# openfheorg/openfhe-development

Measured on AMD Instinct MI355X. Metric: NTT GB/s vs HBM roofline + CKKS EvalMultKeySwitch/sec, N=2^16 L=30, 1/2/4/8 GPU, higher is better.
Workload: dtype u64; 1 GPU; batched fwd+inv negacyclic NTT, N=2^16, L=30 x 60-bit limbs, 1024 polynomials per GPU (BASELINE configs[1]); global_batch=1024, parallelism=batch-sharded x1, no data-path collective

## Files before the change

### openfhe-development_amd/csrc/fhe_hip.cpp

```cpp
#include "../../include/fhe_hip.h"

#include <algorithm>
#include <cmath>
#include <cstdio>
#include <cstdlib>
#include <map>
#include <mutex>
#include <shared_mutex>
#include <string>
#include <vector>

#include "basis_kernels.h"
#include "bfv_kernels.h"
#include "elemwise_kernels.h"
#include "host_math.h"
#include "ntt_kernels.h"
#include "ntt_static.h"
#include "ntt_row8.h"
#include "rt.h"
#include "sampler_kernels.h"
#include "blake2_kernels.h"

using namespace fhe;

static thread_local std::string g_lastError;
static fhe_status fail(fhe_status code, const std::string& msg) {
    g_lastError = msg;
    return code;
}
#define RT_CHECK(expr)                                                                  \
    do {                                                                                \
        const char* _e = (expr);                                                        \
        if (_e)                                                                         \
            return fail(FHE_ERR_DEVICE, std::string(#expr) + ": " + _e);                \
    } while (0)
#define ARG_CHECK(cond, msg)                  \
    do {                                      \
        if (!(cond))                          \
            return fail(FHE_ERR_ARG, msg);    \
    } while (0)

extern "C" const char* fhe_last_error(void) { return g_lastError.c_str(); }
extern "C" const char* fhe_version(void) {
#ifdef FHE_EMU
    return "fhe_hip 0.1 (TEST lane emulator build — not a product build)";
#else
    return "fhe_hip 0.1 (gfx950)";
#endif
}
extern "C" int fhe_device_count(void) { return rt::device_count(); }

namespace fhe {
namespace host {
bool is_prime(uint64_t n) {
    static const uint64_t w[] = {2, 3, 5, 7, 11, 13, 17, 19, 23, 29, 31, 37};
    if (n < 2)
        return false;
    for (uint64_t p : w) {
        if (n == p)
            return true;
        if (n % p == 0)
            return false;
    }
    uint64_t d = n - 1;
    int s      = 0;
    while (!(d & 1)) {
        d >>= 1;
        ++s;
    }
    for (uint64_t a : w) {
        uint64_t x = powmod(a, d, n);
// ... 559 lines not shown
}
static fhe_status launch_pass(const fhe_ctx* c, const PassPlan& pp, bool inverse, const uint64_t* xin, uint64_t* xout,
                              const LimbSel& sel, uint32_t nLimbs, uint32_t batch, bool canonOut, void* stream,
                              uint32_t inStride = 0, uint32_t inFirst = 0, uint32_t outStride = 0, uint32_t outFirst = 0,
                              const NttEpilogue* epi = nullptr, const uint32_t* proSrcLimb = nullptr, int64_t inDelta = 0) {
    NttPassArgs a;
    const uint32_t grid = fill_pass_args(c, pp, inverse, xin, xout, sel, nLimbs, batch, canonOut, inStride, inFirst, outStride,
                                         outFirst, a);
    if (inDelta) {
        if (c->logN < (uint32_t)kTileLog)
            return fail(FHE_ERR_UNSUPPORTED, "ntt: separately allocated towers need a ring of at least 4096");
        a.inDelta = inDelta;
    }
    if (proSrcLimb) {
        a.proMode = 1, a.proSrcLimb = *proSrcLimb;
        const int mode = static_mode(c, pp, inverse);
        if (pp.layoutA && !inverse && mode == 1 && pp.T == 4)
            FHE_LAUNCH_BARRIER((ntt_static_kernel<true, false, 4, 1, false, true>), grid, stream, a);
        else if (pp.layoutA && !inverse && mode == 1 && pp.T == 5)
            FHE_LAUNCH_BARRIER((ntt_static_kernel<true, false, 5, 1, false, true>), grid, stream, a);
        else
            return fail(FHE_ERR_UNSUPPORTED, "ntt: no prologue kernel for this pass shape");
        LAUNCH_CHECK();
        return FHE_OK;
    }
    if (epi && epi->mode) {
        a.epiMode = epi->mode, a.epiSplit = epi->split, a.epiAStride = epi->aStride, a.epiAFirst = epi->aFirst;
        a.epiA = epi->A, a.epiC = epi->C, a.epiOut0 = epi->out0, a.epiOut1 = epi->out1;
        a.epiADelta = epi->aDelta;
        const int mode = static_mode(c, pp, inverse);
        bool launched  = false;
#define FHE_EPI_CASE(TT, MODE) \
    if (!launched && !pp.layoutA && !inverse && pp.T == TT && mode == MODE) { \
        FHE_LAUNCH_BARRIER((ntt_static_kernel<false, false, TT, MODE, true>), grid, stream, a); \
        launched = true; \
    }
        FHE_EPI_CASE(12, 9) FHE_EPI_CASE(11, 9) FHE_EPI_CASE(10, 9) FHE_EPI_CASE(9, 9) FHE_EPI_CASE(12, 1)
#undef FHE_EPI_CASE
        if (!launched)
            return fail(FHE_ERR_UNSUPPORTED, "ntt: no epilogue kernel for this pass shape");
        LAUNCH_CHECK();
        return FHE_OK;
    }
    if (c->logN >= (uint32_t)kTileLog) {
        const int mode = static_mode(c, pp, inverse);
        bool launched  = false;
#define FHE_STATIC_CASE(LA, INV, TT, MODE) \
    if (!launched && pp.layoutA == LA && inverse == INV && pp.T == TT && mode == MODE) { \
        FHE_LAUNCH_BARRIER((ntt_static_kernel<LA, INV, TT, MODE>), grid, stream, a); \
        launched = true; \
    }
        if (!pp.layoutA && c->logN > (uint32_t)kTileLog && row8_for(pp.T)) {
            const uint32_t rgrid = a.rows << (c->logN - pp.T);
            a.xcdSwizzle         = ((nLimbs << (c->logN - pp.T)) % 8u == 0) ? 1u : 0u;
#define FHE_ROW8_CASE(INV, TT, MODE) \
    if (!launched && inverse == INV && pp.T == TT && mode == MODE) { \
        FHE_LAUNCH_BARRIER_N((r8::ntt_row8_kernel<INV, TT - 9, MODE>), rgrid, 64u << (TT - 9), stream, a); \
        launched = true; \
    }
            FHE_ROW8_CASE(false, 12, 9) FHE_ROW8_CASE(true, 12, 0) FHE_ROW8_CASE(false, 11, 9) FHE_ROW8_CASE(true, 11, 0)
            FHE_ROW8_CASE(false, 10, 9) FHE_ROW8_CASE(true, 10, 0) FHE_ROW8_CASE(false, 9, 9) FHE_ROW8_CASE(true, 9, 0)
#undef FHE_ROW8_CASE
        }
        FHE_STATIC_CASE(true, false, 4, 1) FHE_STATIC_CASE(true, true, 4, 1)
        FHE_STATIC_CASE(true, false, 5, 1) FHE_STATIC_CASE(true, true, 5, 1)
        FHE_STATIC_CASE(false, false, 12, 9) FHE_STATIC_CASE(false, true, 12, 0)
        FHE_STATIC_CASE(false, false, 11, 9) FHE_STATIC_CASE(false, true, 11, 0)
        FHE_STATIC_CASE(false, false, 10, 9) FHE_STATIC_CASE(false, true, 10, 0)
        FHE_STATIC_CASE(false, false, 9, 9) FHE_STATIC_CASE(false, true, 9, 0)
        FHE_STATIC_CASE(false, false, 12, 1) FHE_STATIC_CASE(false, true, 12, 1)
#undef FHE_STATIC_CASE
        if (!launched)
            return fail(FHE_ERR_UNSUPPORTED, "ntt: no kernel instance for this pass shape");
        LAUNCH_CHECK();
        return FHE_OK;
    }
    if (pp.layoutA) {
        if (inverse)
            FHE_LAUNCH_BARRIER((ntt_pass_kernel<true, true>), grid, stream, a);
        else
            FHE_LAUNCH_BARRIER((ntt_pass_kernel<true, false>), grid, stream, a);
    }
    else {
        if (inverse)
            FHE_LAUNCH_BARRIER((ntt_pass_kernel<false, true>), grid, stream, a);
        else
            FHE_LAUNCH_BARRIER((ntt_pass_kernel<false, false>), grid, stream, a);
    }
    LAUNCH_CHECK();
    return FHE_OK;
}

static uint32_t env_u32(const char* name, uint32_t dflt) {
    const char* v = std::getenv(name);
    return v ? (uint32_t)std::strtoul(v, nullptr, 10) : dflt;
}
static uint32_t ntt_t1(uint32_t logN) {
    const uint32_t dflt = std::max(4u, logN - (uint32_t)kTileLog);
    static const uint32_t forced = env_u32("FHE_NTT_T1", 0);
    if (forced >= 4 && forced <= 5 && logN > (uint32_t)kTileLog && logN - forced >= 9 && logN - forced <= 12)
        return forced;
    return dflt;
}

static bool ntt_epilogue_supported(const fhe_ctx* c) {
    if (c->logN < (uint32_t)kTileLog)
        return false;
    if (c->logN == (uint32_t)kTileLog)
        return true;
    const uint32_t t1 = ntt_t1(c->logN), t2 = c->logN - t1;
    return t2 == 12u || (t1 == 4u && t2 >= 9u && t2 <= 12u);
}
static bool ntt_prologue_supported(const fhe_ctx* c) {
    return c->logN > (uint32_t)kTileLog && ntt_t1(c->logN) <= 5u;
}
static fhe_status ntt_run(fhe_ctx* c, bool inverse, const uint64_t* xin, uint64_t* xout, const uint32_t* limbIdx,
                          uint32_t nLimbs, uint32_t batch, void* stream, uint32_t inStride = 0, uint32_t inFirst = 0,
                          uint32_t outStride = 0, uint32_t outFirst = 0, const NttEpilogue* epi = nullptr,
                          bool canonOut = true, const uint32_t* proSrcLimb = nullptr, int64_t inDelta = 0) {
    ARG_CHECK(c && xin && xout, "fhe_ntt: null argument");
    ARG_CHECK(batch >= 1, "fhe_ntt: batch must be >= 1");
    LimbSel sel;
    if (fhe_status s = make_sel(c, limbIdx, nLimbs, &sel, "fhe_ntt"))
        return s;
    RT_CHECK(rt::set_device(c->device));
    const uint32_t logN = c->logN;
    if (logN <= (uint32_t)kTileLog) {
        PassPlan p;
        plan_pass(inverse, false, logN, logN, &p);
        uint32_t bound = 1;
        mark_uniform(p, logN);
        if (!inverse)
            schedule_fwd(p, logN, &bound);
        p.outBound = bound;
        return launch_pass(c, p, inverse, xin, xout, sel, nLimbs, batch, canonOut, stream, inStride, inFirst, outStride, outFirst, epi,
                           nullptr, inDelta);
    }
    const uint32_t T1 = ntt_t1(logN), T2 = logN - T1;
    PassPlan pa, pb;
    plan_pass(inverse, true, logN, T1, &pa);
    plan_pass(inverse, false, logN, T2, &pb);
    mark_uniform(pa, logN);
    mark_uniform(pb, logN);
    if (!inverse) {
        uint32_t bound = 1;
        schedule_fwd(pa, logN, &bound);
        schedule_fwd(pb, logN, &bound);
        pb.outBound = bound;
    }
    const PassPlan& p1 = inverse ? pb : pa;
    const PassPlan& p2 = inverse ? pa : pb;
    if (fhe_status s = launch_pass(c, p1, inverse, xin, xout, sel, nLimbs, batch, false, stream, inStride, inFirst, outStride, outFirst,
                                   nullptr, proSrcLimb, inDelta))
        return s;
    return launch_pass(c, p2, inverse, xout, xout, sel, nLimbs, batch, canonOut, stream, outStride, outFirst, outStride, outFirst, epi);
}

extern "C" fhe_status fhe_ntt_fwd(fhe_ctx* c, uint64_t* x, const uint32_t* li, uint32_t nl, uint32_t b, void* st) {
    return ntt_run(c, false, x, x, li, nl, b, st);
}
extern "C" fhe_status fhe_ntt_inv(fhe_ctx* c, uint64_t* x, const uint32_t* li, uint32_t nl, uint32_t b, void* st) {
    return ntt_run(c, true, x, x, li, nl, b, st);
}
extern "C" fhe_status fhe_ntt_fwd_oop(fhe_ctx* c, const uint64_t* xi, uint64_t* xo, const uint32_t* li, uint32_t nl,
                                      uint32_t b, void* st) {
    return ntt_run(c, false, xi, xo, li, nl, b, st);
}
extern "C" fhe_status fhe_ntt_inv_oop(fhe_ctx* c, const uint64_t* xi, uint64_t* xo, const uint32_t* li, uint32_t nl,
                                      uint32_t b, void* st) {
    return ntt_run(c, true, xi, xo, li, nl, b, st);
}

extern "C" size_t fhe_poly_mul_workspace_bytes(const fhe_ctx* c, uint32_t nLimbs, uint32_t batch) {
    return c ? (((size_t)2 * batch * nLimbs) << c->logN) * 8 : 0;
}
static bool poly_mul_fused_supported(const fhe_ctx* c) {
    if (c->logN <= (uint32_t)kTileLog)
        return false;
    const uint32_t t1 = ntt_t1(c->logN), t2 = c->logN - t1;
    return (t1 == 4u && t2 >= 9u && t2 <= 12u) || (t1 == 5u && t2 == 12u);
}
extern "C" fhe_status fhe_poly_mul(fhe_ctx* c, const uint64_t* a, const uint64_t* b, uint64_t* out, const uint32_t* limbIdx,
                                   uint32_t nLimbs, uint32_t batch, void* wsv, size_t wsBytes, void* stream) {
    ARG_CHECK(c && a && b && out && wsv, "fhe_poly_mul: null argument");
    ARG_CHECK(batch >= 1, "fhe_poly_mul: batch must be >= 1");
    ARG_CHECK(wsBytes >= fhe_poly_mul_workspace_bytes(c, nLimbs, batch), "fhe_poly_mul: workspace too small");
    LimbSel sel;
    if (fhe_status s = make_sel(c, limbIdx, nLimbs, &sel, "fhe_poly_mul"))
        return s;
    RT_CHECK(rt::set_device(c->device));
    uint64_t* wa = (uint64_t*)wsv;
    uint64_t* wb = wa + (((size_t)batch * nLimbs) << c->logN);
    if (!poly_mul_fused_supported(c)) {
        if (fhe_status s = ntt_run(c, false, a, wa, limbIdx, nLimbs, batch, stream))
            return s;
        if (fhe_status s = ntt_run(c, false, b, wb, limbIdx, nLimbs, batch, stream))
            return s;
        if (fhe_status s = fhe_mul(c, out, wa, wb, limbIdx, nLimbs, batch, stream))
            return s;
        return ntt_run(c, true, out, out, limbIdx, nLimbs, batch, stream);
    }
    const uint32_t logN = c->logN, T1 = ntt_t1(logN), T2 = logN - T1;
    PassPlan fa, fb, ib, ia;
    plan_pass(false, true, logN, T1, &fa);
    plan_pass(false, false, logN, T2, &fb);
    plan_pass(true, false, logN, T2, &ib);
    plan_pass(true, true, logN, T1, &ia);
// ... 1028 lines not shown
    w.dig.assign(numParts, 0);
    size_t off = 0;
    w.coef = off, off += (size_t)batch * sizeQl * N;
    for (uint32_t j = 0; j < numParts; ++j) {
        const uint32_t start = p->alpha * j;
        const uint32_t sz    = (j == numParts - 1) ? sizeQl - start : p->alpha;
        w.dig[j] = off, off += (size_t)batch * (sizeQl - sz + p->sizeP) * N;
    }
    w.e0 = off, off += (size_t)batch * (sizeQl + p->sizeP) * N;
    w.e1 = off, off += (size_t)batch * (sizeQl + p->sizeP) * N;
    w.md = off, off += (size_t)2 * batch * sizeQl * N;
    w.pcoef = off, off += (size_t)2 * batch * p->sizeP * N;
    w.d2 = off, off += (size_t)batch * sizeQl * N;
    w.k0 = off, off += (size_t)batch * sizeQl * N;
    w.k1 = off, off += (size_t)batch * sizeQl * N;
    w.total = off;
    return w;
}
extern "C" size_t fhe_ks_workspace_bytes(const fhe_ks_plan* p, uint32_t sizeQl, uint32_t batch) {
    if (!p || sizeQl < 1 || sizeQl > p->sizeQ || batch < 1)
        return 0;
    return ks_layout(p, sizeQl, batch).total * 8;
}

static fhe_status mod_down_core(fhe_ks_plan* p, fhe_ks_plan::Level* lv, const uint64_t* x, uint32_t nTow, uint64_t* pcoef,
                                uint64_t* md, void* st, fhe_conv* down = nullptr, const NttEpilogue* epi = nullptr) {
    fhe_ctx* c            = p->ctx;
    const uint32_t sizeQl = lv->sizeQl, sizeP = p->sizeP, sizeQlP = sizeQl + sizeP;
    std::vector<uint32_t> pIdx(sizeP);
    for (uint32_t j = 0; j < sizeP; ++j)
        pIdx[j] = p->sizeQ + j;
    if (fhe_status s = ntt_run(c, true, x, pcoef, pIdx.data(), sizeP, nTow, st, sizeQlP, sizeQl))
        return s;
    if (fhe_status s = fhe_approx_switch_basis(down ? down : lv->down, pcoef, sizeP, 0, md, sizeQl, 0, nTow, st))
        return s;
    return ntt_run(c, false, md, md, nullptr, sizeQl, nTow, st, 0, 0, 0, 0, epi);
}
static fhe_status mod_down_tail(fhe_ks_plan* p, fhe_ks_plan::Level* lv, const uint64_t* x, const uint64_t* md, uint32_t nTow,
                                uint64_t* out, bool accumulate, void* st) {
    const uint32_t sizeQl = lv->sizeQl, sizeQlP = sizeQl + p->sizeP;
    if (accumulate)
        return elem_run<OP_SUB_MUL_CONST_ACC>(p->ctx, out, x, md, lv->d_PInv, nullptr, sizeQl, nTow, st, "fhe_approx_mod_down",
                                              sizeQlP, 0);
    return elem_run<OP_SUB_MUL_CONST>(p->ctx, out, x, md, lv->d_PInv, nullptr, sizeQl, nTow, st, "fhe_approx_mod_down", sizeQlP, 0);
}
static fhe_status mod_down_run(fhe_ks_plan* p, fhe_ks_plan::Level* lv, const uint64_t* x, uint32_t nTow, uint64_t* out,
                               uint64_t* pcoef, uint64_t* md, void* st) {
    if (fhe_status s = mod_down_core(p, lv, x, nTow, pcoef, md, st))
        return s;
    return mod_down_tail(p, lv, x, md, nTow, out, false, st);
}

static fhe_status ks_precompute_run(fhe_ks_plan* p, fhe_ks_plan::Level* lv, const uint64_t* cin, uint32_t batch,
                                    uint64_t* ws, const KsLayout& w, void* st) {
    fhe_ctx* c            = p->ctx;
    const uint32_t sizeQl = lv->sizeQl;
    if (fhe_status s = fhe_ntt_inv_oop(c, cin, ws + w.coef, nullptr, sizeQl, batch, st))
        return s;
    for (uint32_t j = 0; j < lv->numParts; ++j) {
        const uint32_t nc = (uint32_t)lv->cidx[j].size();
        uint64_t* dj      = ws + w.dig[j];
        if (fhe_status s = fhe_approx_switch_basis(lv->up[j], ws + w.coef, sizeQl, p->alpha * j, dj, nc, 0, batch, st))
            return s;
        if (fhe_status s = ntt_run(c, false, dj, dj, lv->cidx[j].data(), nc, batch, st, 0, 0, 0, 0, nullptr, false))
            return s;
    }
    return FHE_OK;
}
static fhe_status ks_inner_multi_launch(fhe_ks_plan* p, fhe_ks_plan::Level* lv, const fhe_ks_key* const* keys, uint32_t nKeys,
                                        const uint64_t* cin, uint32_t batch, uint64_t* const* e0, uint64_t* const* e1,
                                        const uint64_t* first, const TwPair* dP, uint64_t* ws, const KsLayout& w, void* st,
                                        uint32_t towOff = 0) {
    fhe_ctx* c            = p->ctx;
    const uint32_t sizeQl = lv->sizeQl, sizeP = p->sizeP, sizeQlP = sizeQl + sizeP;
    const uint32_t tilesPerRow = c->N >= (uint32_t)kTile ? (c->N >> kTileLog) : 1u;
    for (uint32_t t0 = 0; t0 < nKeys; t0 += (uint32_t)kMaxMultiKeys) {
        KsInnerMultiArgs g;
        const uint32_t nt = std::min<uint32_t>(kMaxMultiKeys, nKeys - t0);
        for (uint32_t j = 0; j < (uint32_t)kMaxDigits; ++j) {
            g.nc[j]     = j < lv->numParts ? (uint32_t)lv->cidx[j].size() : 0u;
            g.digits[j] = j < lv->numParts ? ws + w.dig[j] + (((size_t)towOff * g.nc[j]) << c->logN) : nullptr;
        }
        for (uint32_t t = 0; t < (uint32_t)kMaxMultiKeys; ++t) {
            const uint32_t tt = t < nt ? t0 + t : t0;
            g.keyB[t] = keys[tt]->d_b, g.keyA[t] = keys[tt]->d_a, g.out0[t] = e0[tt], g.out1[t] = e1[tt];
        }
        g.c = cin + (((size_t)towOff * sizeQl) << c->logN), g.first = first, g.firstC = dP;
        g.lc = c->d_lc, g.mu128 = c->d_mu128, g.red = c->d_red;
        g.logN = c->logN, g.batch = batch, g.sizeQl = sizeQl, g.sizeQ = p->sizeQ, g.sizeP = sizeP;
        g.numDigits = lv->numParts, g.alpha = p->alpha, g.nKeys = nt;
        const uint64_t grid = (((uint64_t)tilesPerRow * sizeQlP + 7) / 8) * 8 * batch;
        static const uint32_t ksm = env_u32("FHE_KSM", 1);
        uintptr_t bits = (uintptr_t)g.c | (uintptr_t)g.first;
        for (uint32_t j = 0; j < lv->numParts && j < (uint32_t)kMaxDigits; ++j)
            bits |= (uintptr_t)g.digits[j];
        for (uint32_t t = 0; t < nt; ++t)
            bits |= (uintptr_t)g.keyB[t] | (uintptr_t)g.keyA[t] | (uintptr_t)g.out0[t] | (uintptr_t)g.out1[t];
        const bool wide = (bits & 15u) == 0 && c->N >= 2;
        if (lv->numParts <= 3 && ksm == 1 && wide)
            FHE_LAUNCH((ks_inner_multi_kernel<3, 2, true>), grid, st, g);
        else if (lv->numParts <= 3 && ksm == 2 && wide)
            FHE_LAUNCH((ks_inner_multi_kernel<3, 2, false>), grid, st, g);
        else if (lv->numParts <= 3 && ksm == 3)
            FHE_LAUNCH((ks_inner_multi_kernel<3, 1, false>), grid, st, g);
        else if (lv->numParts <= 3)
            FHE_LAUNCH((ks_inner_multi_kernel<3>), grid, st, g);
        else if (lv->numParts <= 4)
            FHE_LAUNCH((ks_inner_multi_kernel<4>), grid, st, g);
        else
            FHE_LAUNCH((ks_inner_multi_kernel<8>), grid, st, g);
        LAUNCH_CHECK();
    }
    return FHE_OK;
}
static fhe_status ks_inner_run(fhe_ks_plan* p, fhe_ks_plan::Level* lv, const fhe_ks_key* key, const uint64_t* cin,
                               uint32_t batch, uint64_t* e0, uint64_t* e1, uint64_t* ws, const KsLayout& w, void* st,
                               uint32_t towOff = 0) {
// ... 19 lines not shown
    }
    return FHE_OK;
}
static fhe_status ks_inner_multi_run(fhe_ks_plan* p, fhe_ks_plan::Level* lv, const fhe_ks_key* const* keys, uint32_t nKeys,
                                     const uint64_t* cin, uint32_t batch, uint64_t* const* e0, uint64_t* const* e1,
                                     const uint64_t* first, const TwPair* dP, uint64_t* ws, const KsLayout& w, void* st) {
    if (lv->numParts <= (uint32_t)kMaxDigits)
        return ks_inner_multi_launch(p, lv, keys, nKeys, cin, batch, e0, e1, first, dP, ws, w, st);
    const uint32_t sizeQl = lv->sizeQl, sizeQlP = sizeQl + p->sizeP;
    for (uint32_t t = 0; t < nKeys; ++t) {
        if (fhe_status s = ks_inner_run(p, lv, keys[t], cin, batch, e0[t], e1[t], ws, w, st))
            return s;
        if (first)
            if (fhe_status s = elem_run<OP_MUL_CONST_ADD>(p->ctx, e0[t], first, e0[t], dP, nullptr, sizeQl, batch, st,
                                                          "fhe_eval_fast_rotation_ext", 0, 0, sizeQlP, 0, sizeQlP, 0))
                return s;
    }
    return FHE_OK;
}
extern "C" fhe_status fhe_inner_product(fhe_ctx* c, uint32_t nTerms, const uint64_t* const* x, const uint64_t* const* k0,
                                        const uint64_t* const* k1, const uint32_t* keyRow, const uint32_t* limbIdx,
                                        uint32_t rows, uint32_t batch, uint64_t* out0, uint64_t* out1, void* st) {
    ARG_CHECK(c && x && k0 && out0, "fhe_inner_product: null argument");
    ARG_CHECK((k1 != nullptr) == (out1 != nullptr), "fhe_inner_product: the second key and the second output go together");
    ARG_CHECK(batch >= 1, "fhe_inner_product: batch must be >= 1");
    ARG_CHECK(nTerms >= 1, "fhe_inner_product: no terms");
    InnerRowsArgs g;
    if (fhe_status s = make_sel(c, limbIdx, rows, &g.sel, "fhe_inner_product"))
        return s;
    for (uint32_t i = 0; i < (uint32_t)kMaxLimbs; ++i) {
        const uint32_t kr = i < rows ? (keyRow ? keyRow[i] : i) : 0u;
        ARG_CHECK(kr < 256u, "fhe_inner_product: key row out of range");
        g.keyRow[i] = (uint8_t)kr;
    }
    for (uint32_t j = 0; j < nTerms; ++j)
        ARG_CHECK(x[j] && k0[j] && (!k1 || k1[j]), "fhe_inner_product: null term");
    RT_CHECK(rt::set_device(c->device));
    g.out0 = out0, g.out1 = out1, g.lc = c->d_lc, g.mu128 = c->d_mu128;
    g.logN = c->logN, g.batch = batch, g.rows = rows;
    const uint32_t tilesPerRow = c->N >= (uint32_t)kTile ? (c->N >> kTileLog) : 1u;
    for (uint32_t t0 = 0; t0 < nTerms; t0 += (uint32_t)kMaxDigits) {
        const uint32_t nt = std::min<uint32_t>(kMaxDigits, nTerms - t0);
        for (uint32_t j = 0; j < (uint32_t)kMaxDigits; ++j) {
            g.x[j]  = j < nt ? x[t0 + j] : nullptr;
            g.k0[j] = j < nt ? k0[t0 + j] : nullptr;
            g.k1[j] = (j < nt && k1) ? k1[t0 + j] : nullptr;
        }
        g.nTerms = nt, g.acc = t0 > 0;
        FHE_LAUNCH(inner_rows_kernel, (uint64_t)tilesPerRow * rows * batch, st, g);
        LAUNCH_CHECK();
    }
    return FHE_OK;
}
static fhe_status ks_fast_run(fhe_ks_plan* p, fhe_ks_plan::Level* lv, const fhe_ks_key* key, const uint64_t* cin,
                              uint32_t batch, uint64_t* out0, uint64_t* out1, uint64_t* ws, const KsLayout& w, void* st,
                              bool accumulate) {
    fhe_ctx* c            = p->ctx;
    const uint32_t sizeQl = lv->sizeQl;
    if (fhe_status s = ks_inner_run(p, lv, key, cin, batch, ws + w.e0, ws + w.e1, ws, w, st))
        return s;
    if (ntt_epilogue_supported(c)) {
        NttEpilogue epi;
        epi.mode = accumulate ? 2u : 1u, epi.split = batch, epi.aStride = sizeQl + p->sizeP, epi.aFirst = 0;
        epi.A = ws + w.e0, epi.C = lv->d_PInv, epi.out0 = out0, epi.out1 = out1;
        return mod_down_core(p, lv, ws + w.e0, 2 * batch, ws + w.pcoef, ws + w.md, st, nullptr, &epi);
    }
    if (fhe_status s = mod_down_core(p, lv, ws + w.e0, 2 * batch, ws + w.pcoef, ws + w.md, st))
        return s;
    if (fhe_status s = mod_down_tail(p, lv, ws + w.e0, ws + w.md, batch, out0, accumulate, st))
        return s;
    return mod_down_tail(p, lv, ws + w.e1, ws + w.md + ((size_t)batch * sizeQl << c->logN), batch, out1, accumulate, st);
}
static fhe_status keyswitch_run(fhe_ks_plan* p, const fhe_ks_key* key, const uint64_t* cin, uint32_t sizeQl,
                                uint32_t batch, uint64_t* out0, uint64_t* out1, uint64_t* ws, const KsLayout& w,
                                void* st, bool accumulate = false) {
    fhe_ks_plan::Level* lv = nullptr;
    if (fhe_status s = ks_level(p, sizeQl, &lv))
        return s;
    if (fhe_status s = ks_precompute_run(p, lv, cin, batch, ws, w, st))
        return s;
    return ks_fast_run(p, lv, key, cin, batch, out0, out1, ws, w, st, accumulate);
}

extern "C" fhe_status fhe_keyswitch_hybrid(fhe_ks_plan* p, const fhe_ks_key* key, const uint64_t* cin, uint32_t sizeQl,
                                           uint32_t batch, uint64_t* out0, uint64_t* out1, void* ws, size_t wsBytes,
                                           void* st) {
    ARG_CHECK(p && key && cin && out0 && out1 && ws, "fhe_keyswitch_hybrid: null argument");
    ARG_CHECK(key->plan == p, "fhe_keyswitch_hybrid: key belongs to another plan");
    ARG_CHECK(sizeQl >= 1 && sizeQl <= p->sizeQ && batch >= 1, "fhe_keyswitch_hybrid: bad level or batch");
    const KsLayout w = ks_layout(p, sizeQl, batch);
    ARG_CHECK(wsBytes >= w.total * 8, "fhe_keyswitch_hybrid: workspace too small");
    RT_CHECK(rt::set_device(p->ctx->device));
    return keyswitch_run(p, key, cin, sizeQl, batch, out0, out1, (uint64_t*)ws, w, st);
}

extern "C" fhe_status fhe_keyswitch_hybrid_acc(fhe_ks_plan* p, const fhe_ks_key* key, const uint64_t* cin, uint32_t sizeQl,
                                               uint32_t batch, uint64_t* acc0, uint64_t* acc1, void* ws, size_t wsBytes, void* st) {
    ARG_CHECK(p && key && cin && acc0 && acc1 && ws, "fhe_keyswitch_hybrid_acc: null argument");
    ARG_CHECK(key->plan == p, "fhe_keyswitch_hybrid_acc: key belongs to another plan");
    ARG_CHECK(sizeQl >= 1 && sizeQl <= p->sizeQ && batch >= 1, "fhe_keyswitch_hybrid_acc: bad level or batch");
    const KsLayout w = ks_layout(p, sizeQl, batch);
    ARG_CHECK(wsBytes >= w.total * 8, "fhe_keyswitch_hybrid_acc: workspace too small");
    RT_CHECK(rt::set_device(p->ctx->device));
    return keyswitch_run(p, key, cin, sizeQl, batch, acc0, acc1, (uint64_t*)ws, w, st, true);
}

extern "C" fhe_status fhe_ckks_eval_mult(fhe_ks_plan* p, const fhe_ks_key* key, const uint64_t* a0, const uint64_t* a1,
                                         const uint64_t* b0, const uint64_t* b1, uint32_t sizeQl, uint32_t batch,
                                         uint64_t* c0, uint64_t* c1, void* wsv, size_t wsBytes, void* st) {
    ARG_CHECK(p && key && a0 && a1 && b0 && b1 && c0 && c1 && wsv, "fhe_ckks_eval_mult: null argument");
    ARG_CHECK(key->plan == p, "fhe_ckks_eval_mult: key belongs to another plan");
    ARG_CHECK(sizeQl >= 1 && sizeQl <= p->sizeQ && batch >= 1, "fhe_ckks_eval_mult: bad level or batch");
    const KsLayout w = ks_layout(p, sizeQl, batch);
    ARG_CHECK(wsBytes >= w.total * 8, "fhe_ckks_eval_mult: workspace too small");
    fhe_ctx* c   = p->ctx;
    uint64_t* ws = (uint64_t*)wsv;
    RT_CHECK(rt::set_device(c->device));
    if (fhe_status s = fhe_tensor(c, a0, a1, b0, b1, c0, c1, ws + w.d2, nullptr, sizeQl, batch, st))
        return s;
    return keyswitch_run(p, key, ws + w.d2, sizeQl, batch, c0, c1, ws, w, st, true);
}

#define KS_COMMON_CHECKS(who)                                                                              \
    ARG_CHECK(p && ws, who ": null argument");                                                             \
    ARG_CHECK(sizeQl >= 1 && sizeQl <= p->sizeQ && batch >= 1, who ": bad level or batch");                \
    const KsLayout w = ks_layout(p, sizeQl, batch);                                                        \
    ARG_CHECK(wsBytes >= w.total * 8, who ": workspace too small");                                        \
    RT_CHECK(rt::set_device(p->ctx->device));                                                              \
    fhe_ks_plan::Level* lv = nullptr;                                                                      \
    if (fhe_status s_ = ks_level(p, sizeQl, &lv))                                                          \
        return s_;

extern "C" fhe_status fhe_ks_precompute(fhe_ks_plan* p, const uint64_t* c1, uint32_t sizeQl, uint32_t batch, void* ws,
                                        size_t wsBytes, void* st) {
// ... 1226 lines not shown
```

### openfhe-development_amd/csrc/ntt_row8.h

```cpp
#ifndef FHE_NTT_ROW8_H
#define FHE_NTT_ROW8_H
#include "ntt_static.h"
#include "ntt_bfly8_pinned.h"

namespace fhe {
namespace r8 {

constexpr int kRegion = 576;

FHE_HD constexpr uint32_t fc3(uint32_t c) { return 8u * (c & 3u) + 264u * (c >> 2); }
FHE_HD constexpr uint32_t fc4(uint32_t c) { return 8u * (c & 3u) + 288u * (c >> 2); }

template <bool UNI, int B>
FHE_HD void fwd_stage(uint64_t (&r)[8], const TwPair (&w)[4], const BflyConst c, uint32_t (&bnd)[8]) {
#ifdef FHE_PINNED_ASM
    (void)bnd;
    if constexpr (UNI) {
        if constexpr (B == 0) stage_fwd_s_b0(r, w, c);
        if constexpr (B == 1) stage_fwd_s_b1(r, w, c);
        if constexpr (B == 2) stage_fwd_s_b2(r, w, c);
    }
    else {
        if constexpr (B == 0) stage_fwd_v_b0(r, w, c);
        if constexpr (B == 1) stage_fwd_v_b1(r, w, c);
// ... 171 lines not shown
        bnd[k] = 3;
    TwPair w2[4], w1[4], w0[4];
    if constexpr (NB >= 3) load_tw<UNI, 0>(w0, tw, hi, F, logN);
    if constexpr (NB >= 2) load_tw<UNI, 1>(w1, tw, hi, F, logN);
    if constexpr (NB >= 1 && NB < 3) load_tw<UNI, 2>(w2, tw, hi, F, logN);
    if constexpr (NB >= 3) inv_stage<UNI, NB, 0>(r, w0, c, bnd);
    if constexpr (NB >= 3) load_tw<UNI, 2>(w2, tw, hi, F, logN);
    if constexpr (NB >= 2) inv_stage<UNI, NB, 1>(r, w1, c, bnd);
    if constexpr (NB >= 1) inv_stage<UNI, NB, 2>(r, w2, c, bnd);
    if constexpr (!LAZY && NB >= 1)
        inv_end<NB>(r, c, bnd);
}

template <int WB, int BIN>
struct FwdSched {
    static constexpr int TA = WB;
    static constexpr int stages(int i) { return i == 0 ? TA : 3; }
    static constexpr int before(int i) {
        int b = BIN;
        for (int j = 0; j < i; ++j)
            b = (b + 3 * stages(j) <= 16) ? b + 3 * stages(j) : 2 + 3 * stages(j);
        return b;
    }
    static constexpr bool sweep(int i) { return before(i) + 3 * stages(i) > 16; }
    static constexpr int out = before(4);
};

struct TileAt {
    uint32_t tb, rit, tr;
};
FHE_DEV TileAt tile_at(const NttPassArgs& a, uint32_t vt, uint32_t trLog, bool swz) {
    uint32_t tile = vt;
    if (swz) {
        const uint32_t xcd = vt & 7u, i = vt >> 3;
        const uint32_t b = i % a.batch, pairIdx = i / a.batch;
        const uint32_t pair = pairIdx * 8u + xcd;
        tile = ((b * a.nLimbs + (pair >> trLog)) << trLog) + (pair & ((1u << trLog) - 1u));
    }
    const uint32_t row = tile >> trLog;
    return TileAt{row / a.nLimbs, row % a.nLimbs, tile & ((1u << trLog) - 1u)};
}

#if defined(__HIP_DEVICE_COMPILE__)
#define FHE_R8_OPAQUE_V(x) asm volatile("" : "+v"(x))
#else
#define FHE_R8_OPAQUE_V(x) ((void)0)
#endif
#define FHE_R8_LANE()                 \
    uint32_t tq_ = t;                 \
    FHE_R8_OPAQUE_V(tq_);             \
    const uint32_t l = tq_ & 63u, lhi = l >> 3, llo = l & 7u; \
    (void)lhi, (void)llo

template <bool INV, int WB, int MODE>
FHE_DEV void ntt_row8_core(const NttPassArgs& a, uint64_t* lds) {
    static_assert(WB >= 0 && WB <= 3, "row8: 1, 2, 4 or 8 waves per tile");
    static_assert(!(INV && MODE != 0), "row8: the inverse pass that ends a transform is ntt_static.h's");
    constexpr uint32_t tileLog = 9u + (uint32_t)WB;
    constexpr uint32_t threads = 64u << WB;
    constexpr int WLOW         = 3 - WB;
    const uint32_t t     = FHE_TID;
    const uint32_t wv    = WB ? FHE_UNIFORM(t >> 6) : 0u;
    const uint32_t logN  = a.logN;
    const uint32_t trLog = logN - tileLog;
    uint64_t* reg = lds + (size_t)wv * kRegion;
    uint64_t r[8];
    const TileAt at      = tile_at(a, FHE_BID, trLog, a.xcdSwizzle != 0);
    const uint32_t jbase = at.tr << tileLog;
    const uint32_t rit   = at.rit;
    const uint64_t inRow  = a.inStride ? ((uint64_t)at.tb * a.inStride + a.inFirst + rit) : ((uint64_t)at.tb * a.nLimbs + rit);
    const uint64_t outRow = a.outStride ? ((uint64_t)at.tb * a.outStride + a.outFirst + rit) : ((uint64_t)at.tb * a.nLimbs + rit);
    const uint32_t limb = FHE_UNIFORM(a.sel.idx[rit]);
    const uint64_t q    = FHE_ULOAD64(a.q, limb);
    const uint64_t twoq = q << 1, nq = 0 - q;
    const TwPair* tw    = a.tw + ((uint64_t)limb << logN);
    const uint64_t redc = FHE_ULOAD64(a.red, limb);
    const BflyConst c{(uint32_t)nq, (uint32_t)(nq >> 32), q, twoq, 0 - twoq, twoq + q, (uint32_t)redc, (uint32_t)(redc >> 32)};
    const uint64_t* src = (a.inDelta ? a.xin + (int64_t)at.tb * a.inDelta + ((uint64_t)(a.inFirst + rit) << logN) : a.xin + (inRow << logN)) + jbase;
    uint64_t* dst       = a.x + (outRow << logN) + jbase;
    auto x1 = [](int rr) { return (uint32_t)kRegion * ((uint32_t)rr >> WLOW) + (64u << WB) * ((uint32_t)rr & ((1u << WLOW) - 1u)); };

    if constexpr (!INV) {
        using S = FwdSched<WB, (MODE == 9 ? 2 : MODE)>;
        if constexpr (WB > 0) {
            {
                FHE_R8_LANE();
                const uint64_t* s0 = src + tq_;
#pragma unroll
                for (int k = 0; k < 8; ++k)
                    r[k] = FHE_GLD(&s0[threads * (uint32_t)k]);
            }
            fwd_step<true, WB, S::sweep(0)>(r, tw, at.tr, 6 + WB, logN, c, S::sweep(0) ? 2u : (uint32_t)S::before(0));
            FHE_R8_LANE();
            uint64_t* Lw = lds + tq_;
#pragma unroll
            for (int k = 0; k < 8; ++k)
                FHE_LDS_ST(Lw[x1(k)], r[k]);
            FHE_SSYNC();
            const uint64_t* Lr = reg + l;
#pragma unroll
            for (int k = 0; k < 8; ++k)
                FHE_LDS_LD(r[k], Lr[64 * k]);
        }
        else {
            FHE_R8_LANE();
            const uint64_t* s0 = src + l;
#pragma unroll
            for (int k = 0; k < 8; ++k)
                r[k] = FHE_GLD(&s0[64u * (uint32_t)k]);
        }
        fwd_step<true, 3, S::sweep(1)>(r, tw, (jbase >> 9) + wv, 6, logN, c, S::sweep(1) ? 2u : (uint32_t)S::before(1));
        {
            FHE_R8_LANE();
            FHE_WAVE_SYNC();
            uint64_t* Lw = reg + l;
#pragma unroll
            for (int k = 0; k < 8; ++k)
                FHE_LDS_ST(Lw[72 * k], r[k]);
            FHE_WAVE_SYNC();
            const uint64_t* Lr = reg + 72u * lhi + llo;
#pragma unroll
            for (int k = 0; k < 8; ++k)
                FHE_LDS_LD(r[k], Lr[8 * k]);
            fwd_step<false, 3, S::sweep(2)>(r, tw, (jbase >> 6) + (wv << 3) + lhi, 3, logN, c, S::sweep(2) ? 2u : (uint32_t)S::before(2));
        }
        {
            FHE_R8_LANE();
            FHE_WAVE_SYNC();
            uint64_t* Lw = reg + fc3(lhi) + llo;
#pragma unroll
            for (int k = 0; k < 8; ++k)
                FHE_LDS_ST(Lw[33 * k], r[k]);
            FHE_WAVE_SYNC();
            const uint64_t* Lr = reg + fc3(lhi) + 33u * llo;
#pragma unroll
            for (int k = 0; k < 8; ++k)
                FHE_LDS_LD(r[k], Lr[k]);
            fwd_step<false, 3, S::sweep(3)>(r, tw, (jbase >> 3) + (wv << 6) + l, 0, logN, c, S::sweep(3) ? 2u : (uint32_t)S::before(3));
        }
        if (a.canonStep != 0xffffffffu) {
            red_all(r, c);
            csub_all(r, q);
        }
        {
            FHE_R8_LANE();
            FHE_WAVE_SYNC();
            uint64_t* Lw = reg + fc4(lhi) + llo;
#pragma unroll
            for (int k = 0; k < 8; ++k)
                FHE_LDS_ST(Lw[36 * k], r[k]);
            FHE_WAVE_SYNC();
            const uint64_t* Lr = reg + lhi + 36u * llo;
#pragma unroll
            for (int k = 0; k < 8; ++k)
                FHE_LDS_LD(r[k], Lr[fc4((uint32_t)k)]);
            uint64_t* d0 = dst + (wv << 9) + l;
#pragma unroll
            for (int k = 0; k < 8; ++k)
                FHE_GST(&d0[64u * (uint32_t)k], r[k]);
        }
    }
    else {
        {
            FHE_R8_LANE();
            const uint64_t* s0 = src + (wv << 9) + l;
#pragma unroll
            for (int k = 0; k < 8; ++k)
                r[k] = FHE_GLD(&s0[64u * (uint32_t)k]);
            uint64_t* Lw = reg + lhi + 36u * llo;
#pragma unroll
            for (int k = 0; k < 8; ++k)
                FHE_LDS_ST(Lw[fc4((uint32_t)k)], r[k]);
            FHE_WAVE_SYNC();
            const uint64_t* Lr = reg + fc4(lhi) + llo;
#pragma unroll
            for (int k = 0; k < 8; ++k)
                FHE_LDS_LD(r[k], Lr[36 * k]);
            inv_step<false, 3, false>(r, tw, (jbase >> 3) + (wv << 6) + l, 0, logN, c);
        }
        {
            FHE_R8_LANE();
            FHE_WAVE_SYNC();
            uint64_t* Lw = reg + fc3(lhi) + 33u * llo;
#pragma unroll
            for (int k = 0; k < 8; ++k)
                FHE_LDS_ST(Lw[k], r[k]);
            FHE_WAVE_SYNC();
            const uint64_t* Lr = reg + fc3(lhi) + llo;
#pragma unroll
            for (int k = 0; k < 8; ++k)
                FHE_LDS_LD(r[k], Lr[33 * k]);
            inv_step<false, 3, false>(r, tw, (jbase >> 6) + (wv << 3) + lhi, 3, logN, c);
        }
        {
            FHE_R8_LANE();
            FHE_WAVE_SYNC();
            uint64_t* Lw = reg + 72u * lhi + llo;
#pragma unroll
            for (int k = 0; k < 8; ++k)
                FHE_LDS_ST(Lw[8 * k], r[k]);
            FHE_WAVE_SYNC();
            const uint64_t* Lr = reg + l;
#pragma unroll
            for (int k = 0; k < 8; ++k)
                FHE_LDS_LD(r[k], Lr[72 * k]);
        }
        inv_step<true, 3, (WB == 0)>(r, tw, (jbase >> 9) + wv, 6, logN, c);
        if constexpr (WB > 0) {
            FHE_R8_LANE();
            {
                FHE_WAVE_SYNC();
                uint64_t* Lw = reg + l;
#pragma unroll
                for (int k = 0; k < 8; ++k)
                    FHE_LDS_ST(Lw[64 * k], r[k]);
                FHE_SSYNC();
                const uint64_t* Lr = lds + tq_;
#pragma unroll
                for (int k = 0; k < 8; ++k)
                    FHE_LDS_LD(r[k], Lr[x1(k)]);
            }
            inv_step<true, WB, true>(r, tw, at.tr, 6 + WB, logN, c);
            uint64_t* d0 = dst + tq_;
#pragma unroll
            for (int k = 0; k < 8; ++k)
                FHE_GST(&d0[threads * (uint32_t)k], r[k]);
        }
        else {
            FHE_R8_LANE();
            uint64_t* d0 = dst + l;
#pragma unroll
            for (int k = 0; k < 8; ++k)
                FHE_GST(&d0[64u * (uint32_t)k], r[k]);
        }
    }
}
#undef FHE_R8_LANE

template <bool INV, int WB, int MODE>
FHE_GLOBAL void FHE_LAUNCH_BOUNDS2(64 << WB, 8) ntt_row8_kernel(const NttPassArgs a) {
    FHE_SHARED_U64(lds, (1 << WB) * kRegion);
    ntt_row8_core<INV, WB, MODE>(a, lds);
}

}
}
#endif
```

Before: 2278 GB/s.

## Fuse digit row-NTT pass with key inner product in hybrid keyswitch

Adds a fused keyswitch kernel. It performs the final row pass of the forward NTT on each digit tile in registers, then multiplies by the key-switch key with 128-bit accumulation, reduces, and writes both outputs directly. The precompute NTT now stops after its column pass when fusion applies. This is meant to remove the write and re-read of the NTT'd digits and a separate inner-product kernel. The row-pass code is refactored into a shared helper, and the row8 launch uses a copy of the args so the swizzle flag no longer leaks into other launches. It risks register pressure from the 16 128-bit accumulators.

```diff
diff --git a/openfhe-development_amd/csrc/fhe_hip.cpp b/openfhe-development_amd/csrc/fhe_hip.cpp
--- a/openfhe-development_amd/csrc/fhe_hip.cpp
+++ b/openfhe-development_amd/csrc/fhe_hip.cpp
@@ -17,6 +17,7 @@
 #include "ntt_kernels.h"
 #include "ntt_static.h"
 #include "ntt_row8.h"
+#include "ks_fused.h"
 #include "rt.h"
 #include "sampler_kernels.h"
 #include "blake2_kernels.h"
@@ -682,10 +683,11 @@
     }
         if (!pp.layoutA && c->logN > (uint32_t)kTileLog && row8_for(pp.T)) {
             const uint32_t rgrid = a.rows << (c->logN - pp.T);
-            a.xcdSwizzle         = ((nLimbs << (c->logN - pp.T)) % 8u == 0) ? 1u : 0u;
+            NttPassArgs a8       = a;
+            a8.xcdSwizzle        = ((nLimbs << (c->logN - pp.T)) % 8u == 0) ? 1u : 0u;
 #define FHE_ROW8_CASE(INV, TT, MODE) \
     if (!launched && inverse == INV && pp.T == TT && mode == MODE) { \
-        FHE_LAUNCH_BARRIER_N((r8::ntt_row8_kernel<INV, TT - 9, MODE>), rgrid, 64u << (TT - 9), stream, a); \
+        FHE_LAUNCH_BARRIER_N((r8::ntt_row8_kernel<INV, TT - 9, MODE>), rgrid, 64u << (TT - 9), stream, a8); \
         launched = true; \
     }
             FHE_ROW8_CASE(false, 12, 9) FHE_ROW8_CASE(true, 12, 0) FHE_ROW8_CASE(false, 11, 9) FHE_ROW8_CASE(true, 11, 0)
@@ -747,7 +749,7 @@
 static fhe_status ntt_run(fhe_ctx* c, bool inverse, const uint64_t* xin, uint64_t* xout, const uint32_t* limbIdx,
                           uint32_t nLimbs, uint32_t batch, void* stream, uint32_t inStride = 0, uint32_t inFirst = 0,
                           uint32_t outStride = 0, uint32_t outFirst = 0, const NttEpilogue* epi = nullptr,
-                          bool canonOut = true, const uint32_t* proSrcLimb = nullptr, int64_t inDelta = 0) {
+                          bool canonOut = true, const uint32_t* proSrcLimb = nullptr, int64_t inDelta = 0, uint32_t columnOnlyT1 = 0) {
     ARG_CHECK(c && xin && xout, "fhe_ntt: null argument");
     ARG_CHECK(batch >= 1, "fhe_ntt: batch must be >= 1");
     LimbSel sel;
@@ -766,7 +768,7 @@
         return launch_pass(c, p, inverse, xin, xout, sel, nLimbs, batch, canonOut, stream, inStride, inFirst, outStride, outFirst, epi,
                            nullptr, inDelta);
     }
-    const uint32_t T1 = ntt_t1(logN), T2 = logN - T1;
+    const uint32_t T1 = columnOnlyT1 ? columnOnlyT1 : ntt_t1(logN), T2 = logN - T1;
     PassPlan pa, pb;
     plan_pass(inverse, true, logN, T1, &pa);
     plan_pass(inverse, false, logN, T2, &pb);
@@ -783,6 +785,8 @@
     if (fhe_status s = launch_pass(c, p1, inverse, xin, xout, sel, nLimbs, batch, false, stream, inStride, inFirst, outStride, outFirst,
                                    nullptr, proSrcLimb, inDelta))
         return s;
+    if (columnOnlyT1)
+        return inverse ? fail(FHE_ERR_UNSUPPORTED, "ntt: only a forward transform stops after its column pass") : FHE_OK;
     return launch_pass(c, p2, inverse, xout, xout, sel, nLimbs, batch, canonOut, stream, outStride, outFirst, outStride, outFirst, epi);
 }
 
@@ -1917,7 +1921,7 @@
 }
 
 static fhe_status ks_precompute_run(fhe_ks_plan* p, fhe_ks_plan::Level* lv, const uint64_t* cin, uint32_t batch,
-                                    uint64_t* ws, const KsLayout& w, void* st) {
+                                    uint64_t* ws, const KsLayout& w, void* st, uint32_t columnOnlyT1 = 0) {
     fhe_ctx* c            = p->ctx;
     const uint32_t sizeQl = lv->sizeQl;
     if (fhe_status s = fhe_ntt_inv_oop(c, cin, ws + w.coef, nullptr, sizeQl, batch, st))
@@ -1927,7 +1931,7 @@
         uint64_t* dj      = ws + w.dig[j];
         if (fhe_status s = fhe_approx_switch_basis(lv->up[j], ws + w.coef, sizeQl, p->alpha * j, dj, nc, 0, batch, st))
             return s;
-        if (fhe_status s = ntt_run(c, false, dj, dj, lv->cidx[j].data(), nc, batch, st, 0, 0, 0, 0, nullptr, false))
+        if (fhe_status s = ntt_run(c, false, dj, dj, lv->cidx[j].data(), nc, batch, st, 0, 0, 0, 0, nullptr, false, nullptr, 0, columnOnlyT1))
             return s;
     }
     return FHE_OK;
@@ -2053,12 +2057,51 @@
     }
     return FHE_OK;
 }
+static uint32_t ks_fused_t2(const fhe_ks_plan* p, const fhe_ks_plan::Level* lv, const fhe_ks_key* key, const uint64_t* cin,
+                            const uint64_t* ws) {
+    static const uint32_t on = env_u32("FHE_KS_FUSED", 1);
+    const fhe_ctx* c = p->ctx;
+    if (!on || c->logN <= (uint32_t)kTileLog || lv->numParts > (uint32_t)r8::kFusedDigits)
+        return 0;
+    uint32_t t2 = c->logN - ntt_t1(c->logN);
+    if (t2 == 12u && c->logN - 11u <= 5u)
+        t2 = 11u;
+    if (t2 < 9u || t2 > 12u)
+        return 0;
+    return (((uintptr_t)cin | (uintptr_t)ws | (uintptr_t)key->d_b | (uintptr_t)key->d_a) & 15u) == 0 ? t2 : 0;
+}
+static fhe_status ks_fused_run(fhe_ks_plan* p, fhe_ks_plan::Level* lv, const fhe_ks_key* key, const uint64_t* cin, uint32_t batch,
+                               uint64_t* e0, uint64_t* e1, uint64_t* ws, const KsLayout& w, void* st, uint32_t t2) {
+    fhe_ctx* c = p->ctx;
+    r8::KsFusedArgs g;
+    for (uint32_t j = 0; j < (uint32_t)r8::kFusedDigits; ++j) {
+        g.nc[j]     = j < lv->numParts ? (uint32_t)lv->cidx[j].size() : 0u;
+        g.digits[j] = j < lv->numParts ? ws + w.dig[j] : nullptr;
+    }
+    g.c = cin, g.keyB = key->d_b, g.keyA = key->d_a, g.out0 = e0, g.out1 = e1;
+    g.tw = c->d_tw, g.q = c->d_q, g.red = c->d_red, g.lc = c->d_lc, g.mu128 = c->d_mu128;
+    g.logN = c->logN, g.batch = batch, g.sizeQl = lv->sizeQl, g.sizeQ = p->sizeQ, g.sizeP = p->sizeP;
+    g.numDigits = lv->numParts, g.alpha = p->alpha;
+    const uint64_t groups = ((uint64_t)(lv->sizeQl + p->sizeP) << (c->logN - t2));
+    const uint64_t grid   = (groups + 7) / 8 * 8 * batch;
+    if (t2 == 12u)
+        FHE_LAUNCH_BARRIER_N((r8::ks_fused_kernel<3>), grid, 512u, st, g);
+    else if (t2 == 11u)
+        FHE_LAUNCH_BARRIER_N((r8::ks_fused_kernel<2>), grid, 256u, st, g);
+    else if (t2 == 10u)
+        FHE_LAUNCH_BARRIER_N((r8::ks_fused_kernel<1>), grid, 128u, st, g);
+    else
+        FHE_LAUNCH_BARRIER_N((r8::ks_fused_kernel<0>), grid, 64u, st, g);
+    LAUNCH_CHECK();
+    return FHE_OK;
+}
 static fhe_status ks_fast_run(fhe_ks_plan* p, fhe_ks_plan::Level* lv, const fhe_ks_key* key, const uint64_t* cin,
                               uint32_t batch, uint64_t* out0, uint64_t* out1, uint64_t* ws, const KsLayout& w, void* st,
-                              bool accumulate) {
+                              bool accumulate, uint32_t fusedT2 = 0) {
     fhe_ctx* c            = p->ctx;
     const uint32_t sizeQl = lv->sizeQl;
-    if (fhe_status s = ks_inner_run(p, lv, key, cin, batch, ws + w.e0, ws + w.e1, ws, w, st))
+    if (fhe_status s = fusedT2 ? ks_fused_run(p, lv, key, cin, batch, ws + w.e0, ws + w.e1, ws, w, st, fusedT2)
+                               : ks_inner_run(p, lv, key, cin, batch, ws + w.e0, ws + w.e1, ws, w, st))
         return s;
     if (ntt_epilogue_supported(c)) {
         NttEpilogue epi;
@@ -2078,9 +2121,10 @@
     fhe_ks_plan::Level* lv = nullptr;
     if (fhe_status s = ks_level(p, sizeQl, &lv))
         return s;
-    if (fhe_status s = ks_precompute_run(p, lv, cin, batch, ws, w, st))
-        return s;
-    return ks_fast_run(p, lv, key, cin, batch, out0, out1, ws, w, st, accumulate);
+    const uint32_t fusedT2 = ks_fused_t2(p, lv, key, cin, ws);
+    if (fhe_status s = ks_precompute_run(p, lv, cin, batch, ws, w, st, fusedT2 ? p->ctx->logN - fusedT2 : 0u))
+        return s;
+    return ks_fast_run(p, lv, key, cin, batch, out0, out1, ws, w, st, accumulate, fusedT2);
 }
 
 extern "C" fhe_status fhe_keyswitch_hybrid(fhe_ks_plan* p, const fhe_ks_key* key, const uint64_t* cin, uint32_t sizeQl,
diff --git a/openfhe-development_amd/csrc/ks_fused.h b/openfhe-development_amd/csrc/ks_fused.h
--- /dev/null
+++ b/openfhe-development_amd/csrc/ks_fused.h
@@ -0,0 +1,149 @@
+#ifndef FHE_KS_FUSED_H
+#define FHE_KS_FUSED_H
+#include "basis_kernels.h"
+#include "ntt_row8.h"
+
+namespace fhe {
+namespace r8 {
+
+constexpr int kFusedDigits = 3;
+struct KsFusedArgs {
+    const uint64_t* c;
+    const uint64_t* digits[kFusedDigits];
+    const uint64_t* keyB;
+    const uint64_t* keyA;
+    uint64_t* out0;
+    uint64_t* out1;
+    const TwPair* tw;
+    const uint64_t* q;
+    const uint64_t* red;
+    const LimbConst* lc;
+    const uint64_t* mu128;
+    uint32_t logN, batch, sizeQl, sizeQ, sizeP, numDigits, alpha;
+    uint32_t nc[kFusedDigits];
+};
+
+FHE_HD void mac128(u128w& s, uint64_t a, uint64_t b) {
+    const uint32_t al = (uint32_t)a, ah = (uint32_t)(a >> 32), bl = (uint32_t)b, bh = (uint32_t)(b >> 32);
+    const uint64_t p0 = mul32x32(al, bl);
+    const uint64_t p1 = mad64(al, bh, p0 >> 32);
+    const uint64_t p2 = mad64(ah, bl, (uint32_t)p1);
+    const uint64_t hi = mad64(ah, bh, p1 >> 32) + (p2 >> 32);
+    const uint64_t lo = (p0 & 0xffffffffull) | (p2 << 32);
+    s.lo += lo;
+    s.hi += hi + (s.lo < lo);
+}
+
+FHE_DEV uint32_t tid_fresh(uint32_t wv) {
+#if defined(__HIP_DEVICE_COMPILE__)
+    uint32_t l;
+    asm volatile("v_mbcnt_lo_u32_b32 %0, -1, 0\n\tv_mbcnt_hi_u32_b32 %0, -1, %0" : "=v"(l));
+    return (wv << 6) | l;
+#else
+    (void)wv;
+    return FHE_TID;
+#endif
+}
+
+template <int WB>
+FHE_DEV void ks_fused_core(const KsFusedArgs& g, uint64_t* lds) {
+    static_assert(WB >= 0 && WB <= 3, "ks_fused: 1, 2, 4 or 8 waves per tile");
+    constexpr uint32_t tileLog = 9u + (uint32_t)WB;
+    const uint32_t t           = FHE_TID;
+    const uint32_t wv          = WB ? FHE_UNIFORM(t >> 6) : 0u;
+    const uint32_t logN        = g.logN;
+    const uint32_t tilesPerRow = 1u << (logN - tileLog);
+    const uint32_t sizeQlP     = g.sizeQl + g.sizeP;
+    const uint32_t xcd = FHE_BID & 7u, slot = FHE_BID >> 3;
+    const uint32_t b   = slot % g.batch;
+    const uint32_t grp = (slot / g.batch) * 8u + xcd;
+    const uint32_t tr  = grp & (tilesPerRow - 1u);
+    const uint32_t i   = grp >> (logN - tileLog);
+    if (i >= sizeQlP)
+        return;
+    const uint32_t idx   = FHE_UNIFORM(i < g.sizeQl ? i : i + (g.sizeQ - g.sizeQl));
+    const uint64_t q     = FHE_ULOAD64(g.q, idx);
+    const uint64_t twoq  = q << 1, nq = 0 - q;
+    const uint64_t redc  = FHE_ULOAD64(g.red, idx);
+    const BflyConst c{(uint32_t)nq, (uint32_t)(nq >> 32), q, twoq, 0 - twoq, twoq + q, (uint32_t)redc, (uint32_t)(redc >> 32)};
+    const TwPair* tw     = g.tw + ((uint64_t)idx << logN);
+    const uint32_t jbase = tr << tileLog;
+    uint64_t* reg        = lds + (size_t)wv * kRegion;
+    const uint32_t mBase = jbase + (wv << 9);
+#define FHE_KSF_LANE_OFF()   \
+    const uint32_t lo_ = (tid_fresh(wv) & 63u) << 3
+
+    u128w s0[8], s1[8];
+#pragma unroll
+    for (int m = 0; m < 8; ++m)
+        s0[m] = s1[m] = u128w{0, 0};
+    for (uint32_t j = 0; j < g.numDigits; ++j) {
+        const uint32_t start = j * g.alpha;
+        const uint32_t sz    = sizeQlP - g.nc[j];
+        const bool own       = i >= start && i < start + sz;
+        uint64_t r[8];
+        if (own) {
+            FHE_KSF_LANE_OFF();
+            const uint64_t* p = g.c + (((uint64_t)b * g.sizeQl + i) << logN) + mBase + lo_;
+#pragma unroll
+            for (int m = 0; m < 8; m += 2) {
+                uint64_t v[2];
+                ld_cpl<2>(p + m, v);
+                r[m] = v[0], r[m + 1] = v[1];
+            }
+        }
+        else {
+            const uint32_t pos = i < start ? i : i - sz;
+            const uint64_t* src = g.digits[j] + (((uint64_t)b * g.nc[j] + pos) << logN) + jbase;
+            if (j) {
+                if constexpr (WB > 0)
+                    FHE_SSYNC();
+                else
+                    FHE_WAVE_SYNC();
+            }
+            fwd_tile_regs<WB, 2>(r, src, tw, tr, jbase, wv, tid_fresh(wv), logN, c, lds, reg);
+            red_all(r, c);
+            csub_all(r, q);
+        }
+        const uint64_t koff = (((uint64_t)j * (g.sizeQ + g.sizeP) + idx) << logN) + mBase;
+        FHE_KSF_LANE_OFF();
+        const uint64_t* kB = g.keyB + koff + lo_;
+        const uint64_t* kA = g.keyA + koff + lo_;
+#pragma unroll
+        for (int m = 0; m < 8; m += 2) {
+            uint64_t vb[2], va[2];
+            ld_cpl<2>(kB + m, vb);
+            ld_cpl<2>(kA + m, va);
+            mac128(s0[m], r[m], vb[0]);
+            mac128(s0[m + 1], r[m + 1], vb[1]);
+            mac128(s1[m], r[m], va[0]);
+            mac128(s1[m + 1], r[m + 1], va[1]);
+        }
+    }
+    const LimbConst lc  = g.lc[idx];
+    const uint64_t mulo = FHE_ULOAD64(g.mu128, 2 * idx), muhi = FHE_ULOAD64(g.mu128, 2 * idx + 1);
+    FHE_KSF_LANE_OFF();
+    const uint64_t ooff = (((uint64_t)b * sizeQlP + i) << logN) + mBase + lo_;
+#pragma unroll
+    for (int m = 0; m < 8; m += 2) {
+        uint64_t v0[2], v1[2];
+#pragma unroll
+        for (int u = 0; u < 2; ++u) {
+            v0[u] = sum8_reduce(sum8{s0[m + u].lo, 0, s0[m + u].hi, 0}, q, lc.msb, mulo, muhi);
+            v1[u] = sum8_reduce(sum8{s1[m + u].lo, 0, s1[m + u].hi, 0}, q, lc.msb, mulo, muhi);
+        }
+        st_cpl<2>(g.out0 + ooff + m, v0);
+        st_cpl<2>(g.out1 + ooff + m, v1);
+    }
+#undef FHE_KSF_LANE_OFF
+}
+
+template <int WB>
+FHE_GLOBAL void FHE_LAUNCH_BOUNDS2(64 << WB, 4) ks_fused_kernel(const KsFusedArgs g) {
+    FHE_SHARED_U64(lds, (1 << WB) * kRegion);
+    ks_fused_core<WB>(g, lds);
+}
+
+}
+}
+#endif
diff --git a/openfhe-development_amd/csrc/ntt_row8.h b/openfhe-development_amd/csrc/ntt_row8.h
--- a/openfhe-development_amd/csrc/ntt_row8.h
+++ b/openfhe-development_amd/csrc/ntt_row8.h
@@ -247,13 +247,81 @@
     const uint32_t l = tq_ & 63u, lhi = l >> 3, llo = l & 7u; \
     (void)lhi, (void)llo
 
+template <int WB>
+FHE_HD constexpr uint32_t x1_word(int rr) {
+    return (uint32_t)kRegion * ((uint32_t)rr >> (3 - WB)) + (64u << WB) * ((uint32_t)rr & ((1u << (3 - WB)) - 1u));
+}
+template <int WB, int BIN>
+FHE_DEV void fwd_tile_regs(uint64_t (&r)[8], const uint64_t* src, const TwPair* tw, uint32_t tr, uint32_t jbase, uint32_t wv, uint32_t t,
+                           uint32_t logN, const BflyConst c, uint64_t* lds, uint64_t* reg) {
+    constexpr uint32_t threads = 64u << WB;
+    (void)threads;
+    using S = FwdSched<WB, BIN>;
+    if constexpr (WB > 0) {
+        {
+            FHE_R8_LANE();
+            const uint64_t* s0 = src + tq_;
+#pragma unroll
+            for (int k = 0; k < 8; ++k)
+                r[k] = FHE_GLD(&s0[threads * (uint32_t)k]);
+        }
+        fwd_step<true, WB, S::sweep(0)>(r, tw, tr, 6 + WB, logN, c, S::sweep(0) ? 2u : (uint32_t)S::before(0));
+        FHE_R8_LANE();
+        uint64_t* Lw = lds + tq_;
+#pragma unroll
+        for (int k = 0; k < 8; ++k)
+            FHE_LDS_ST(Lw[x1_word<WB>(k)], r[k]);
+        FHE_SSYNC();
+        const uint64_t* Lr = reg + l;
+#pragma unroll
+        for (int k = 0; k < 8; ++k)
+            FHE_LDS_LD(r[k], Lr[64 * k]);
+    }
+    else {
+        FHE_R8_LANE();
+        const uint64_t* s0 = src + l;
+#pragma unroll
+        for (int k = 0; k < 8; ++k)
+            r[k] = FHE_GLD(&s0[64u * (uint32_t)k]);
+    }
+    fwd_step<true, 3, S::sweep(1)>(r, tw, (jbase >> 9) + wv, 6, logN, c, S::sweep(1) ? 2u : (uint32_t)S::before(1));
+    {
+        FHE_R8_LANE();
+        FHE_WAVE_SYNC();
+        uint64_t* Lw = reg + l;
+#pragma unroll
+        for (int k = 0; k < 8; ++k)
+            FHE_LDS_ST(Lw[72 * k], r[k]);
+        FHE_WAVE_SYNC();
+        const uint64_t* Lr = reg + 72u * lhi + llo;
+#pragma unroll
+        for (int k = 0; k < 8; ++k)
+            FHE_LDS_LD(r[k], Lr[8 * k]);
+        fwd_step<false, 3, S::sweep(2)>(r, tw, (jbase >> 6) + (wv << 3) + lhi, 3, logN, c, S::sweep(2) ? 2u : (uint32_t)S::before(2));
+    }
+    {
+        FHE_R8_LANE();
+        FHE_WAVE_SYNC();
+        uint64_t* Lw = reg + fc3(lhi) + llo;
+#pragma unroll
+        for (int k = 0; k < 8; ++k)
+            FHE_LDS_ST(Lw[33 * k], r[k]);
+        FHE_WAVE_SYNC();
+        const uint64_t* Lr = reg + fc3(lhi) + 33u * llo;
+#pragma unroll
+        for (int k = 0; k < 8; ++k)
+            FHE_LDS_LD(r[k], Lr[k]);
+        fwd_step<false, 3, S::sweep(3)>(r, tw, (jbase >> 3) + (wv << 6) + l, 0, logN, c, S::sweep(3) ? 2u : (uint32_t)S::before(3));
+    }
+}
+
 template <bool INV, int WB, int MODE>
 FHE_DEV void ntt_row8_core(const NttPassArgs& a, uint64_t* lds) {
     static_assert(WB >= 0 && WB <= 3, "row8: 1, 2, 4 or 8 waves per tile");
     static_assert(!(INV && MODE != 0), "row8: the inverse pass that ends a transform is ntt_static.h's");
     constexpr uint32_t tileLog = 9u + (uint32_t)WB;
     constexpr uint32_t threads = 64u << WB;
-    constexpr int WLOW         = 3 - WB;
+    (void)threads;
     const uint32_t t     = FHE_TID;
     const uint32_t wv    = WB ? FHE_UNIFORM(t >> 6) : 0u;
     const uint32_t logN  = a.logN;
@@ -273,66 +341,9 @@
     const BflyConst c{(uint32_t)nq, (uint32_t)(nq >> 32), q, twoq, 0 - twoq, twoq + q, (uint32_t)redc, (uint32_t)(redc >> 32)};
     const uint64_t* src = (a.inDelta ? a.xin + (int64_t)at.tb * a.inDelta + ((uint64_t)(a.inFirst + rit) << logN) : a.xin + (inRow << logN)) + jbase;
     uint64_t* dst       = a.x + (outRow << logN) + jbase;
-    auto x1 = [](int rr) { return (uint32_t)kRegion * ((uint32_t)rr >> WLOW) + (64u << WB) * ((uint32_t)rr & ((1u << WLOW) - 1u)); };
 
     if constexpr (!INV) {
-        using S = FwdSched<WB, (MODE == 9 ? 2 : MODE)>;
-        if constexpr (WB > 0) {
-            {
-                FHE_R8_LANE();
-                const uint64_t* s0 = src + tq_;
-#pragma unroll
-                for (int k = 0; k < 8; ++k)
-                    r[k] = FHE_GLD(&s0[threads * (uint32_t)k]);
-            }
-            fwd_step<true, WB, S::sweep(0)>(r, tw, at.tr, 6 + WB, logN, c, S::sweep(0) ? 2u : (uint32_t)S::before(0));
-            FHE_R8_LANE();
-            uint64_t* Lw = lds + tq_;
-#pragma unroll
-            for (int k = 0; k < 8; ++k)
-                FHE_LDS_ST(Lw[x1(k)], r[k]);
-            FHE_SSYNC();
-            const uint64_t* Lr = reg + l;
-#pragma unroll
-            for (int k = 0; k < 8; ++k)
-                FHE_LDS_LD(r[k], Lr[64 * k]);
-        }
-        else {
-            FHE_R8_LANE();
-            const uint64_t* s0 = src + l;
-#pragma unroll
-            for (int k = 0; k < 8; ++k)
-                r[k] = FHE_GLD(&s0[64u * (uint32_t)k]);
-        }
-        fwd_step<true, 3, S::sweep(1)>(r, tw, (jbase >> 9) + wv, 6, logN, c, S::sweep(1) ? 2u : (uint32_t)S::before(1));
-        {
-            FHE_R8_LANE();
-            FHE_WAVE_SYNC();
-            uint64_t* Lw = reg + l;
-#pragma unroll
-            for (int k = 0; k < 8; ++k)
-                FHE_LDS_ST(Lw[72 * k], r[k]);
-            FHE_WAVE_SYNC();
-            const uint64_t* Lr = reg + 72u * lhi + llo;
-#pragma unroll
-            for (int k = 0; k < 8; ++k)
-                FHE_LDS_LD(r[k], Lr[8 * k]);
-            fwd_step<false, 3, S::sweep(2)>(r, tw, (jbase >> 6) + (wv << 3) + lhi, 3, logN, c, S::sweep(2) ? 2u : (uint32_t)S::before(2));
-        }
-        {
-            FHE_R8_LANE();
-            FHE_WAVE_SYNC();
-            uint64_t* Lw = reg + fc3(lhi) + llo;
-#pragma unroll
-            for (int k = 0; k < 8; ++k)
-                FHE_LDS_ST(Lw[33 * k], r[k]);
-            FHE_WAVE_SYNC();
-            const uint64_t* Lr = reg + fc3(lhi) + 33u * llo;
-#pragma unroll
-            for (int k = 0; k < 8; ++k)
-                FHE_LDS_LD(r[k], Lr[k]);
-            fwd_step<false, 3, S::sweep(3)>(r, tw, (jbase >> 3) + (wv << 6) + l, 0, logN, c, S::sweep(3) ? 2u : (uint32_t)S::before(3));
-        }
+        fwd_tile_regs<WB, (MODE == 9 ? 2 : MODE)>(r, src, tw, at.tr, jbase, wv, t, logN, c, lds, reg);
         if (a.canonStep != 0xffffffffu) {
             red_all(r, c);
             csub_all(r, q);
@@ -413,7 +424,7 @@
                 const uint64_t* Lr = lds + tq_;
 #pragma unroll
                 for (int k = 0; k < 8; ++k)
-                    FHE_LDS_LD(r[k], Lr[x1(k)]);
+                    FHE_LDS_LD(r[k], Lr[x1_word<WB>(k)]);
             }
             inv_step<true, WB, true>(r, tw, at.tr, 6 + WB, logN, c);
             uint64_t* d0 = dst + tq_;
```

Result: no change. 2275 GB/s (-0.1%).
